# awslabs/palace

Measured on AMD Instinct MI355X. Metric: curl-curl Mult DOF/s + PCG iters/s, p=3 H(curl) 10M DOF @1/2/4/8 GPU, higher is better.
Workload: dtype f64

## Files before the change

palace_amd/csrc/pa_capi.hip:

```cpp
#include <algorithm>
#include <atomic>
#include <cmath>
#include <cstdlib>
#include <cstring>

#include "pa_hex_core.hpp"

namespace pa {

static thread_local std::string g_error;
void set_error(const std::string &msg) { g_error = msg; }

static void require_device() {
  int n = 0;
  const hipError_t err = hipGetDeviceCount(&n);
  if (err != hipSuccess || n == 0)
    throw Error(std::string("no HIP device visible: libpalace_amd has no CPU fallback (hipGetDeviceCount: ") +
                hipGetErrorString(err) + ", " + std::to_string(n) + " devices)");
}

void parse_coeff(const void *blob, size_t bytes, int dim, CoeffHost &out, size_t slot_offset) {
  const size_t nslots = bytes / 8;
  const unsigned char *base = static_cast<const unsigned char *>(blob);
  auto slot_int = [&](size_t i) {
// ... 1171 lines not shown

int pa_op_mult_essential(pa_op *op, const double *x, double *y, void *stream) {
  return guarded([&] {
    PA_REQUIRE(op && op->has_essential, "pa_op_set_essential has not been called");
    apply(op, x, y, true, (hipStream_t)stream, true);
  });
}

int pa_op_mult_essential_diag(pa_op *op, const double *x, double *y, int diag_policy, void *stream, int *handled) {
  return guarded([&] {
    PA_REQUIRE(op && op->has_essential && handled, "pa_op_set_essential has not been called");
    if (op->subs.empty() && op->msubs.empty() && op->dsubs.size() == 1 && op->dsubs[0]->d_ess_flag && x != y &&
        !TransposeScope::active()) {
      const DenseSub &ds = *op->dsubs[0];
      launch_dense_apply(ds, x, true, (hipStream_t)stream);
      launch_dense_gather(ds, y, false, (hipStream_t)stream, nullptr, nullptr, x, diag_policy ? 1 : 0);
      *handled = 1;
      return;
    }
    const SubOp *s0 = op->subs.size() == 1 ? op->subs[0] : nullptr;
    const bool fuse = s0 && op->dsubs.empty() && op->msubs.empty() &&
                      (s0->fe_type == PA_FE_HCURL  ? nd_hex_fuses_essential(*s0)
                       : s0->fe_type == PA_FE_HDIV ? s0->d_shared_bc != nullptr
                                                   : (s0->d_idxc && s0->stream_default && s0->d_perm_s_bc));
    apply(op, x, y, true, (hipStream_t)stream, true, fuse ? (diag_policy ? 1 : 0) : -1);
    *handled = fuse ? 1 : 0;
  });
}

int pa_op_prepare_fused_step(pa_op *op, int *available) {
  return guarded([&] {
    PA_REQUIRE(op && available, "null argument");
    *available = 0;
    const bool enabled = !(getenv("PALACE_AMD_FUSED_STEP") && atoi(getenv("PALACE_AMD_FUSED_STEP")) == 0);
    if (!enabled || !op->has_essential || !op->msubs.empty()) return;
    if (op->subs.empty() && op->dsubs.size() == 1) {
      *available = dense_fused_step_ok(*op->dsubs[0]) ? 1 : 0;
      return;
    }
    if (op->subs.empty() && op->dsubs.size() > 1) {
      const char *e = getenv("PALACE_AMD_FUSED_STEP_SURFACE");
      if ((e && e[0] == '0') || !dense_fused_step_ok(*op->dsubs[0]) || op->dsubs[0]->d_rows) return;
      for (size_t k = 1; k < op->dsubs.size(); k++)
        if (!op->dsubs[k]->d_rows || !op->dsubs[k]->d_idx_bc) return;
      if (!op->d_t_extra) {
        std::vector<int32_t> rows;
        for (size_t k = 1; k < op->dsubs.size(); k++) {
          std::vector<int32_t> r((size_t)op->dsubs[k]->n_rows);
          if (!r.empty()) PA_HIP(hipMemcpy(r.data(), op->dsubs[k]->d_rows, r.size() * sizeof(int32_t), hipMemcpyDeviceToHost));
          rows.insert(rows.end(), r.begin(), r.end());
        }
        std::sort(rows.begin(), rows.end());
        rows.erase(std::unique(rows.begin(), rows.end()), rows.end());
        op->n_extra_rows = (int)rows.size();
        op->d_extra_rows = dev_upload(rows.data(), std::max<size_t>(rows.size(), 1));
        if (op->dsubs.size() - 1 <= (size_t)kMaxSurfaceBlocks) {
          std::vector<int32_t> uptr(rows.size() + 1, 0), uent;
          std::vector<uint8_t> ublk;
          std::vector<std::vector<int32_t>> tptr(op->dsubs.size()), tent(op->dsubs.size());
          for (size_t k = 1; k < op->dsubs.size(); k++) {
            const DenseSub &d = *op->dsubs[k];
            tptr[k].resize((size_t)d.lsize + 1), tent[k].resize((size_t)d.ne * d.P);
            PA_HIP(hipMemcpy(tptr[k].data(), d.d_tptr, tptr[k].size() * sizeof(int32_t), hipMemcpyDeviceToHost));
            PA_HIP(hipMemcpy(tent[k].data(), d.d_tent, tent[k].size() * sizeof(int32_t), hipMemcpyDeviceToHost));
          }
          for (size_t i = 0; i < rows.size(); i++) {
            for (size_t k = 1; k < op->dsubs.size(); k++)
              for (int32_t a = tptr[k][(size_t)rows[i]]; a < tptr[k][(size_t)rows[i] + 1]; a++) uent.push_back(tent[k][(size_t)a]), ublk.push_back((uint8_t)(k - 1));
            uptr[i + 1] = (int32_t)uent.size();
          }
          op->d_urow_ptr = dev_upload(uptr.data(), uptr.size());
          op->d_uent = dev_upload(uent.data(), std::max<size_t>(uent.size(), 1));
          op->d_ublk = dev_upload(ublk.data(), std::max<size_t>(ublk.size(), 1));
        }
        op->d_t_extra = dev_alloc<double>((size_t)op->height);
        PA_HIP(hipMemset(op->d_t_extra, 0, sizeof(double) * (size_t)op->height));
      }
      *available = 1;
      return;
    }
    if (op->subs.size() != 1 || !op->dsubs.empty()) return;
    SubOp *so = op->subs[0];
    if (so->fe_type == PA_FE_H1) {
      if (!so->d_idxc || !so->stream_default || !so->d_perm_s_bc || !h1_hex_stream_ok(*so)) return;
    } else if (so->fe_type != PA_FE_HCURL || (so->q1d != 4 && so->q1d != 5) || !so->d_idxc || !so->d_perm_s_bc || !nd_hex_stream_ok(*so)) {
      return;
    }
    *available = stream_build_all(*so) ? 1 : 0;
  });
}

static const double *dense_surface_terms(pa_op *op, const double *x, hipStream_t s) {
  if (op->dsubs.size() < 2) return nullptr;
  PA_REQUIRE(op->d_t_extra, "pa_op_prepare_fused_step has not been called (or found no fused form)");
  if (op->d_urow_ptr) {
    SurfaceYe ye{};
    for (size_t k = 1; k < op->dsubs.size(); k++) {
      launch_dense_apply(*op->dsubs[k], x, true, s);
      ye.ye[k - 1] = op->dsubs[k]->d_ye;
    }
    launch_surface_rows(op->d_extra_rows, op->n_extra_rows, op->d_urow_ptr, op->d_uent, op->d_ublk, ye, op->d_t_extra, s);
    return op->d_t_extra;
  }
  launch_zero_rows(op->d_t_extra, op->d_extra_rows, op->n_extra_rows, s);
  for (size_t k = 1; k < op->dsubs.size(); k++) {
    launch_dense_apply(*op->dsubs[k], x, true, s);
    launch_dense_gather(*op->dsubs[k], op->d_t_extra, true, s);
  }
  return op->d_t_extra;
}

int pa_op_mult_cheb_step(pa_op *op, const double *x, const pa_cheb_step *step, int diag_policy, void *stream) {
  return guarded([&] {
    PA_REQUIRE(op && x && step && step->dinv && step->r0 && step->out, "null argument");
    PA_REQUIRE(x != step->out, "the step cannot overwrite its own input");
    PA_REQUIRE(!TransposeScope::active() || op->symmetric(), "transposed step of a non-symmetric operator");
    if (op->subs.empty() && !op->dsubs.empty() && dense_fused_step_ok(*op->dsubs[0])) {
      const DenseSub &ds = *op->dsubs[0];
      const double *t_add = dense_surface_terms(op, x, (hipStream_t)stream);
      launch_dense_apply(ds, x, true, (hipStream_t)stream);
      launch_dense_gather_step(ds, x, GatherStep{step->sd, step->sr, step->dinv, step->r0, step->e_prev, step->out, step->add, nullptr, 1,
                                                nullptr, nullptr, t_add},
                               diag_policy ? 1 : 0, (hipStream_t)stream);
      return;
    }
    PA_REQUIRE(op->subs.size() == 1 && op->subs[0]->n_all > 0, "pa_op_prepare_fused_step has not been called (or found no fused form)");
    const SubOp &so = *op->subs[0];
    launch_nd_hex_stream_all(so, x, (hipStream_t)stream);
    launch_et_run_gather_step(so, x, GatherStep{step->sd, step->sr, step->dinv, step->r0, step->e_prev, step->out, step->add, nullptr, 1},
                              diag_policy ? 1 : 0, (hipStream_t)stream);
  });
}

int pa_op_mult_residual(pa_op *op, const double *y, const double *b, double *res, const double *dinv, double c0, double *d0,
                        int diag_policy, void *stream) {
  return guarded([&] {
    PA_REQUIRE(op && y && b && (res || d0) && (!d0 || dinv), "null argument");
    PA_REQUIRE(y != res && y != d0, "the residual cannot overwrite the operator's input");
    PA_REQUIRE(!TransposeScope::active() || op->symmetric(), "transposed step of a non-symmetric operator");
    if (op->subs.empty() && !op->dsubs.empty() && dense_fused_step_ok(*op->dsubs[0])) {
      const DenseSub &ds = *op->dsubs[0];
      const double *t_add = dense_surface_terms(op, y, (hipStream_t)stream);
      launch_dense_apply(ds, y, true, (hipStream_t)stream);
      launch_dense_gather_step(ds, y, GatherStep{0.0, c0, dinv, b, nullptr, d0, 0, res, 2, nullptr, nullptr, t_add}, diag_policy ? 1 : 0,
                               (hipStream_t)stream);
      return;
    }
    PA_REQUIRE(op->subs.size() == 1 && op->subs[0]->n_all > 0, "pa_op_prepare_fused_step has not been called (or found no fused form)");
    const SubOp &so = *op->subs[0];
    launch_nd_hex_stream_all(so, y, (hipStream_t)stream);
    launch_et_run_gather_step(so, y, GatherStep{0.0, c0, dinv, b, nullptr, d0, 0, res, 2}, diag_policy ? 1 : 0, (hipStream_t)stream);
  });
}

int pa_op_supports_split(const pa_op *op) {
  if (!op || !op->msubs.empty()) return 0;
  if (op->subs.size() == 1 && op->dsubs.empty()) {
    const SubOp &so = *op->subs[0];
    return (nd_hex_stream_split_ok(so) || (so.fe_type == PA_FE_H1 && so.d_idxc)) ? 1 : 0;
  }
  if (op->subs.empty() && op->dsubs.size() == 1) return dense_split_ok(*op->dsubs[0]) ? 1 : 0;
  return 0;
}

int pa_op_mult_split(pa_op *op, const double *x, const double *xg0, const double *xg1, const unsigned long long *sel, double *y,
                     double *yg, int n_true, int ess_policy, void *stream) {
  return guarded([&] {
// ... 1 lines not shown
    PA_REQUIRE(pa_op_supports_split(op), "the operator has no split-vector form (pa_op_supports_split)");
    PA_REQUIRE(x != y, "in-place apply is not supported");
    PA_REQUIRE(!TransposeScope::active() || op->symmetric(), "transposed split apply of a non-symmetric operator");
    const bool masked = ess_policy >= 0;
    const SplitIO io{n_true, xg0, xg1, sel, yg};
    hipStream_t s = (hipStream_t)stream;
    if (!op->dsubs.empty()) {
      DenseSub *ds = op->dsubs[0];
      PA_REQUIRE(!masked || op->has_essential, "pa_op_set_essential has not been called");
      launch_dense_apply(*ds, x, masked, s, &io);
      launch_dense_gather(*ds, y, false, s, nullptr, &io, x, ess_policy);
      return;
    }
    SubOp *so = op->subs[0];
    PA_REQUIRE(!masked || (op->has_essential && so->d_perm_s_bc), "pa_op_set_essential has not been called");
    if (so->fe_type == PA_FE_H1)
      launch_h1_hex_stream(*so, x, y, masked, s, &io);
    else
      launch_nd_hex_stream(*so, x, y, masked, s, &io);
    launch_et_run_gather(*so, y, false, s, x, masked, ess_policy, nullptr, &io);
  });
}

int pa_op_mult_split_step(pa_op *op, const double *x, const double *xg0, const double *xg1, const unsigned long long *sel, double *yg,
                          int n_true, int ess_policy, const pa_split_step *st, void *stream) {
  return guarded([&] {
    PA_REQUIRE(op && x && xg0 && yg && st && st->r0 && st->iface_mask && st->t_iface, "null argument");
    PA_REQUIRE(st->mode == 1 ? (st->dinv && st->out) : (st->mode == 2 && (st->res || st->out) && (!st->out || st->dinv)), "invalid step");
    PA_REQUIRE(x != st->out && x != st->res, "the step cannot overwrite the operator's input");
    PA_REQUIRE(!TransposeScope::active() || op->symmetric(), "transposed split apply of a non-symmetric operator");
    PA_REQUIRE(ess_policy < 0 || op->has_essential, "pa_op_set_essential has not been called");
    const SplitIO io{n_true, xg0, xg1, sel, yg};
    hipStream_t s = (hipStream_t)stream;
    if (op->subs.empty() && op->dsubs.size() == 1 && dense_fused_step_ok(*op->dsubs[0]) && dense_split_ok(*op->dsubs[0])) {
      const DenseSub &ds = *op->dsubs[0];
      launch_dense_apply(ds, x, ess_policy >= 0, s, &io);
      launch_dense_gather_step(ds, x, GatherStep{st->sd, st->sr, st->dinv, st->r0, st->e_prev, st->out, st->add, st->res, st->mode,
                                                 st->iface_mask, st->t_iface}, ess_policy, s, &io);
      return;
    }
    PA_REQUIRE(op->subs.size() == 1 && op->dsubs.empty() && op->subs[0]->n_all > 0,
               "pa_op_prepare_fused_step has not been called (or found no fused form)");
    const SubOp &so = *op->subs[0];
    launch_nd_hex_stream_all(so, x, s, &io);
    launch_et_run_gather_step(so, x, GatherStep{st->sd, st->sr, st->dinv, st->r0, st->e_prev, st->out, st->add, st->res, st->mode,
                                                st->iface_mask, st->t_iface}, ess_policy, s, &io);
  });
}

int pa_op_mult2(pa_op *op, const double *x0, const double *x1, double *y0, double *y1, void *stream) {
  return guarded([&] { apply2(op, x0, x1, y0, y1, (hipStream_t)stream, false, -1); });
}

int pa_op_mult2_essential_diag(pa_op *op, const double *x0, const double *x1, double *y0, double *y1, int diag_policy,
                               void *stream, int *handled) {
  return guarded([&] {
    PA_REQUIRE(op && op->has_essential && handled, "pa_op_set_essential has not been called");
    *handled = apply2(op, x0, x1, y0, y1, (hipStream_t)stream, true, diag_policy ? 1 : 0) ? 1 : 0;
  });
}

int pa_op_assemble_diagonal(pa_op *op, double *diag, void *stream) {
  return guarded([&] {
    PA_REQUIRE(op && diag, "null argument");
    PA_REQUIRE(op->msubs.empty(), "mixed-space operators have no diagonal");
    PA_HIP(hipMemsetAsync(diag, 0, sizeof(double) * (size_t)op->height, (hipStream_t)stream));
    for (const SubOp *so : op->subs) {
      if (so->fe_type == PA_FE_HCURL)
        launch_nd_hex_diag(*so, diag, (hipStream_t)stream);
      else if (so->fe_type == PA_FE_HDIV)
        launch_rt_hex_diag(*so, diag, (hipStream_t)stream);
      else
        launch_h1_hex_diag(*so, diag, (hipStream_t)stream);
    }
    for (const DenseSub *ds : op->dsubs) launch_dense_diag(*ds, diag, (hipStream_t)stream);
  });
}

int pa_op_stream_affine(const pa_op *op, int32_t out[3]) {
  return guarded([&] {
    PA_REQUIRE(op && out, "null argument");
    out[0] = out[1] = out[2] = 0;
    for (const SubOp *so : op->subs)
      if (so->fe_type == PA_FE_HCURL && so->qd) {
        out[0] = so->ne, out[1] = so->qd->n_aff_elems, out[2] = so->qd->d_aff ? so->qd->n_aff_batch_elems : 0;
        return;
      }
  });
}
int pa_op_dense_gather_form(const pa_op *op, int32_t out[2]) {
  return guarded([&] {
    PA_REQUIRE(op && out, "null argument");
    out[0] = out[1] = 0;
    if (!op->dsubs.empty()) out[0] = op->dsubs[0]->ye_rows ? 1 : 0, out[1] = dense_gather_group(*op->dsubs[0]);
  });
}
int pa_op_num_sub(const pa_op *op) { return op ? (int)(op->subs.size() + op->dsubs.size() + op->msubs.size()) : -1; }
int pa_op_destroy_assembly_data(const pa_op *op) {
  return guarded([&] { PA_REQUIRE(op, "null operator"); });
}
int pa_op_height(const pa_op *op) { return op ? op->height : -1; }
int pa_op_width(const pa_op *op) { return op ? op->width : -1; }

double pa_op_algorithmic_bytes(const pa_op *op) {
  if (!op) return 0.0;
  double bytes = 0.0;
  for (const SubOp *so : op->subs) {
    if (so->fe_type == PA_FE_HDIV) {
      const bool use_v = so->qf != PA_QF_L2_1;
      const int rows = so->qd ? so->qd->ncomp : (use_v ? 11 : 2);
      bytes += (double)so->ne * ((double)so->Q * rows * 8 + (double)so->P * 6);
      continue;
    }
    bytes += (double)so->ne * ((double)so->Q * 11 * 8 + (double)so->P * (so->fe_type == PA_FE_H1 ? 4 : 5));
  }
  for (const DenseSub *ds : op->dsubs)
    bytes += (double)ds->ne * ((double)ds->Q * ds->geom->nrows * 8 + (double)ds->P * (ds->d_co ? 7 : 5));
  for (const MixedSub *ms : op->msubs)
    if (ms->hex1) bytes += (double)ms->ne * ((double)ms->Q * 11 * 8 + (double)(ms->hex1->P + ms->hex2->P) * 6);
  return bytes + 8.0 * op->height + 8.0 * op->width;
}

void pa_op_destroy(pa_op *op) {
  if (!op) return;
  for (SubOp *so : op->subs) free_sub(so);
  for (DenseSub *ds : op->dsubs) free_dense_sub(ds);
  for (MixedSub *ms : op->msubs) free_mixed_sub(ms);
  (void)hipFree(op->d_t_extra), (void)hipFree(op->d_extra_rows);
  (void)hipFree(op->d_urow_ptr), (void)hipFree(op->d_uent), (void)hipFree(op->d_ublk);
  delete op;
}

}
```

palace_amd/csrc/pa_h1_hex_stream.hip:

```cpp
#include <string>

#include "pa_hex_core.hpp"

namespace pa {

namespace {

using streamhost::kIdxWords;
constexpr int kIdxStart0 = streamhost::kIdxStart0H1;

constexpr int kH1StreamWaves = 2;

template <int P1>
struct H1StreamTab {
  double Bc[2 * (P1 + 1)];
  double Gc[2 * (P1 + 1)];
};

template <int P1>
struct H1StreamArgs {
  int ne, nbatch, chunk;
  const uint32_t *idxc;
  const uint32_t *perm;
  const double *qdata;
  const double *x;
  double *y, *ye;
  int nsplit;
  const double *xg0, *xg1;
  const unsigned long long *xg_sel;
  double *yg;
  H1StreamTab<P1> tab;
};

template <int P1, bool USE_V, bool USE_G, int MINW, bool SPLIT = false>
__global__ __launch_bounds__(64 * kH1StreamWaves, MINW) void h1_hex_stream_kernel(const H1StreamArgs<P1> a) {
  using L = H1Layout<P1, 4>;
  constexpr int Q1 = 4, NC = P1 + 1, PP = NC * NC * NC, NPL = (PP + 15) / 16, NPK = (NPL + 3) / 4;
  constexpr int NG = (USE_V ? 1 : 0) + (USE_G ? 6 : 0);
  constexpr int LDS_SIDE = (PP + 1) / 2 + (NPK + 1) * 8;
  constexpr int LDS_ELEM = (L::ELEM_PAD + LDS_SIDE + 14 + 15) / 32 * 32 + 16;
  extern __shared__ __attribute__((aligned(16))) double smem[];
  const int lane = threadIdx.x & 63;
  const int wave = __builtin_amdgcn_readfirstlane(threadIdx.x >> 6);
  const int xcd = blockIdx.x & 7;
  const int base = xcd * a.chunk, bend = min(base + a.chunk, a.nbatch);
  const int stride = (int)(gridDim.x >> 3) * kH1StreamWaves;
  int b = base + (int)(blockIdx.x >> 3) * kH1StreamWaves + wave;
  if (b >= bend) return;
  const double *Bc = a.tab.Bc, *Gc = a.tab.Gc;
  const double *xgh = nullptr;
  if (SPLIT) xgh = ((a.xg_sel ? *a.xg_sel : 0ull) & 1ull) ? a.xg1 : a.xg0;

  auto load_idx = [&](const int bb, const int sub, const int t, int (&s)[NPL + 2], unsigned (&p)[NPK + 1]) {
    const int e = bb * 4 + sub;
    const uint32_t *ic = a.idxc + (size_t)e * kIdxWords;
#pragma unroll
    for (int r = 0; r < NPL; r++) s[r] = (int)__builtin_nontemporal_load(&ic[r]);
    s[NPL] = (int)__builtin_nontemporal_load(&ic[kIdxStart0 + t]);
    s[NPL + 1] = (int)__builtin_nontemporal_load(&ic[kIdxStart0 + 16 + min(t, 11)]);
    const uint32_t *pp = a.perm + (size_t)e * ((NPK + 1) * 16) + t;
#pragma unroll
    for (int k = 0; k <= NPK; k++) p[k] = __builtin_nontemporal_load(&pp[16 * k]);
  };
  auto gather = [&](int (&s)[NPL + 2], const unsigned (&p)[NPK + 1], double (&xv)[NPL], int *stab, const int t) {
    stab[t] = s[NPL];
    if (t < 12) stab[16 + t] = s[NPL + 1];
    wave_sync();
    const unsigned fw = p[NPK];
#pragma unroll
    for (int r = 0; r < NPL; r++) {
      const unsigned w = (unsigned)s[r], low = (w & 0xffffu) & ((2u << t) - 1u);
      const int rid = (int)((w >> 16) & 31u) + __popc(low) - 1;
      const int pos = low ? 16 * r + 31 - __clz((int)low) : (int)((w >> 21) & 255u);
      int dof = stab[rid] + (t + 16 * r - pos);
      if (!(16 * r + 15 < PP) && t + 16 * r >= PP) dof = 0;
      xv[r] = SPLIT ? (dof < a.nsplit ? a.x : xgh)[dof] : a.x[dof];
      s[r] = dof | ((fw >> (2 * r + 1)) & 1u ? kExclBit : 0) | ((fw >> (18 + r)) & 1u ? kEssBit : 0);
    }
  };
  auto settle = [&](unsigned (&p)[NPK + 1]) {
#pragma unroll
    for (int k = 0; k <= NPK; k++) asm volatile("" : "+v"(p[k]));
  };
  int sA[NPL + 2];
  unsigned pA[NPK + 1];
  double xv[NPL];
  load_idx(b, lane >> 4, lane & 15, sA, pA);
  gather(sA, pA, xv, reinterpret_cast<int *>(smem + (size_t)(wave * 4 + (lane >> 4)) * LDS_ELEM + L::ELEM_PAD + LDS_SIDE), lane & 15);
#pragma unroll
  for (int r = 0; r < NPL; r++) asm volatile("" : "+v"(xv[r]));
  settle(pA);

  for (;;) {
    int lo = lane;
    asm volatile("" : "+v"(lo));
    const int sub = lo >> 4, t = lo & 15, ta = t & 3, tb = t >> 2;
    double *sm = smem + (size_t)(wave * 4 + sub) * LDS_ELEM;
    int *side = reinterpret_cast<int *>(sm + L::ELEM_PAD);
    int *stab = side + 2 * LDS_SIDE;
    const int e = b * 4 + sub;

    double gd[Q1][NG > 0 ? NG : 1];
    {
      const double *g = a.qdata + (size_t)e * NG * 64 + t;
#pragma unroll
      for (int qz = 0; qz < Q1; qz++)
#pragma unroll
        for (int c = 0; c < NG; c++) gd[qz][c] = __builtin_nontemporal_load(&g[c * 64 + 16 * qz]);
    }
    const int bn = b + stride;
    const bool more = bn < bend;
    int sB[NPL + 2];
    unsigned pB[NPK + 1];
    load_idx(more ? bn : b, sub, t, sB, pB);
    __builtin_amdgcn_sched_barrier(0);

#pragma unroll
    for (int r = 0; r < NPL; r++) {
      if (16 * r + 15 < PP || t + 16 * r < PP) {
        const int sv = sA[r];
        sm[(pA[r >> 2] >> (8 * (r & 3))) & 255u] = (sv & kEssBit) ? 0.0 : xv[r];
        side[t + 16 * r] = sv;
      }
    }
#pragma unroll
    for (int k = 0; k <= NPK; k++) side[2 * ((PP + 1) / 2) + 16 * k + t] = (int)pA[k];
    wave_sync();
    double u[NC];
    {
      const bool act = ta < NC && tb < NC;
#pragma unroll
      for (int i = 0; i < NC; i++) u[i] = act ? sm[i + NC * (ta + NC * tb)] : 0.0;
    }
    wave_sync();

    double V[Q1], GV[3][Q1];
    {
      const bool act = ta < NC && tb < NC;
#pragma unroll
      for (int qx = 0; qx < Q1; qx++) {
        double v = 0.0, d = 0.0;
#pragma unroll
        for (int i = 0; i < NC; i++) {
          v += half_even<NC, Q1>(Bc, qx, i) * u[i];
          if (USE_G) d += half_odd<NC, Q1>(Gc, qx, i) * u[i];
        }
        if (act) {
          sm[L::ia(0, qx, ta, tb)] = v;
          if (USE_G) sm[L::ia(1, qx, ta, tb)] = d;
        }
      }
    }
    wave_sync();
    {
      const bool act = tb < NC;
      double v[NC], d[NC];
#pragma unroll
      for (int j = 0; j < NC; j++) {
        v[j] = sm[L::ia(0, ta, j, act ? tb : 0)];
        if (USE_G) d[j] = sm[L::ia(1, ta, j, act ? tb : 0)];
      }
#pragma unroll
      for (int qy = 0; qy < Q1; qy++) {
        double vv = 0.0, vd = 0.0, dv = 0.0;
#pragma unroll
        for (int j = 0; j < NC; j++) {
          vv += half_even<NC, Q1>(Bc, qy, j) * v[j];
          if (USE_G) vd += half_odd<NC, Q1>(Gc, qy, j) * v[j];
          if (USE_G) dv += half_even<NC, Q1>(Bc, qy, j) * d[j];
        }
        if (act) {
          sm[L::ib(0, ta, qy, tb)] = vv;
          if (USE_G) sm[L::ib(1, ta, qy, tb)] = vd, sm[L::ib(2, ta, qy, tb)] = dv;
        }
      }
    }
    wave_sync();
    {
      double vv[NC], vd[NC], dv[NC];
#pragma unroll
      for (int k = 0; k < NC; k++) {
        vv[k] = sm[L::ib(0, ta, tb, k)];
        if (USE_G) vd[k] = sm[L::ib(1, ta, tb, k)], dv[k] = sm[L::ib(2, ta, tb, k)];
      }
#pragma unroll
      for (int qz = 0; qz < Q1; qz++) {
        double val = 0.0, dz = 0.0, dy = 0.0, dx = 0.0;
#pragma unroll
        for (int k = 0; k < NC; k++) {
          if (USE_V) val += half_even<NC, Q1>(Bc, qz, k) * vv[k];
          if (USE_G) {
            dz += half_odd<NC, Q1>(Gc, qz, k) * vv[k];
            dy += half_even<NC, Q1>(Bc, qz, k) * vd[k];
            dx += half_even<NC, Q1>(Bc, qz, k) * dv[k];
          }
        }
        V[qz] = val, GV[0][qz] = dx, GV[1][qz] = dy, GV[2][qz] = dz;
      }
    }
    wave_sync();

#pragma unroll
    for (int qz = 0; qz < Q1; qz++) {
      if (USE_V) V[qz] *= gd[qz][0];
      if (USE_G) sym_mv(&gd[qz][USE_V ? 1 : 0], GV[0][qz], GV[1][qz], GV[2][qz], GV[0][qz], GV[1][qz], GV[2][qz]);
    }

    {
#pragma unroll
      for (int k = 0; k < NC; k++) {
        double vv = 0.0, vd = 0.0, dv = 0.0;
#pragma unroll
        for (int qz = 0; qz < Q1; qz++) {
          if (USE_V) vv += half_even<NC, Q1>(Bc, qz, k) * V[qz];
          if (USE_G) {
            vv += half_odd<NC, Q1>(Gc, qz, k) * GV[2][qz];
            vd += half_even<NC, Q1>(Bc, qz, k) * GV[1][qz];
            dv += half_even<NC, Q1>(Bc, qz, k) * GV[0][qz];
          }
        }
        sm[L::ib(0, ta, tb, k)] = vv;
        if (USE_G) sm[L::ib(1, ta, tb, k)] = vd, sm[L::ib(2, ta, tb, k)] = dv;
      }
    }
    wave_sync();
    double xB[NPL];
    __builtin_amdgcn_sched_barrier(0);
    gather(sB, pB, xB, stab, t);
    settle(pB);
    __builtin_amdgcn_sched_barrier(0);
    {
      const bool act = tb < NC;
      double vv[Q1], vd[Q1], dv[Q1];
#pragma unroll
      for (int qy = 0; qy < Q1; qy++) {
        vv[qy] = sm[L::ib(0, ta, qy, act ? tb : 0)];
        if (USE_G) vd[qy] = sm[L::ib(1, ta, qy, act ? tb : 0)], dv[qy] = sm[L::ib(2, ta, qy, act ? tb : 0)];
      }
#pragma unroll
      for (int j = 0; j < NC; j++) {
        double v = 0.0, d = 0.0;
#pragma unroll
        for (int qy = 0; qy < Q1; qy++) {
          v += half_even<NC, Q1>(Bc, qy, j) * vv[qy];
          if (USE_G) v += half_odd<NC, Q1>(Gc, qy, j) * vd[qy];
          if (USE_G) d += half_even<NC, Q1>(Bc, qy, j) * dv[qy];
        }
        if (act) {
          sm[L::ia(0, ta, j, tb)] = v;
          if (USE_G) sm[L::ia(1, ta, j, tb)] = d;
        }
      }
    }
    wave_sync();
    {
      const bool act = ta < NC && tb < NC;
      double v[Q1], d[Q1];
#pragma unroll
      for (int qx = 0; qx < Q1; qx++) {
        v[qx] = sm[L::ia(0, qx, act ? ta : 0, act ? tb : 0)];
        if (USE_G) d[qx] = sm[L::ia(1, qx, act ? ta : 0, act ? tb : 0)];
      }
#pragma unroll
      for (int i = 0; i < NC; i++) {
        double r = 0.0;
#pragma unroll
        for (int qx = 0; qx < Q1; qx++) {
          r += half_even<NC, Q1>(Bc, qx, i) * v[qx];
          if (USE_G) r += half_odd<NC, Q1>(Gc, qx, i) * d[qx];
        }
        u[i] = r;
      }
    }
    wave_sync();
    {
      const bool act = ta < NC && tb < NC;
#pragma unroll
      for (int i = 0; i < NC; i++)
        if (act) sm[i + NC * (ta + NC * tb)] = u[i];
    }
    wave_sync();
#pragma unroll
    for (int r = 0; r < NPL; r++) {
      const int m = (16 * r + 15 < PP) ? t + 16 * r : min(t + 16 * r, PP - 1), mt = m & 15, mr = m >> 4;
      const unsigned fl = (unsigned)side[2 * ((PP + 1) / 2) + 16 * NPK + mt] >> (2 * mr);
      const double v = sm[((unsigned)side[2 * ((PP + 1) / 2) + 16 * (mr >> 2) + mt] >> (8 * (mr & 3))) & 255u];
      const int d = side[m] & (kExclBit - 1);
      double *yd = a.y;
      if (SPLIT) yd = d < a.nsplit ? a.y : a.yg;
      double *dst = (fl & 2u) ? yd + d : a.ye + ((size_t)e * PP + m);
      *dst = v;
    }
    wave_sync();
    if (!more) break;
    b = bn;
#pragma unroll
    for (int r = 0; r < NPL; r++) sA[r] = sB[r], xv[r] = xB[r];
#pragma unroll
    for (int k = 0; k <= NPK; k++) pA[k] = pB[k];
  }
}

int device_cus_h1() {
  static int cus = [] {
    int dev = 0, n = 0;
    if (hipGetDevice(&dev) != hipSuccess || hipDeviceGetAttribute(&n, hipDeviceAttributeMultiprocessorCount, dev) != hipSuccess || n <= 0)
      n = 256;
    return n;
  }();
  return cus;
}

template <int P1, bool V, bool G, bool SPLIT = false>
void launch_vg(const SubOp &so, H1StreamArgs<P1> &a, hipStream_t s) {
  using L = H1Layout<P1, 4>;
  constexpr int MINW = 3;
  constexpr int NC = P1 + 1, PP = NC * NC * NC, NPL = (PP + 15) / 16, NPK = (NPL + 3) / 4;
  for (int i = 0; i < 2 * NC; i++) a.tab.Bc[i] = so.Bc[i], a.tab.Gc[i] = so.Gc[i];
  const size_t lds = sizeof(double) * (size_t)(kH1StreamWaves * 4) * ((L::ELEM_PAD + (PP + 1) / 2 + (NPK + 1) * 8 + 14 + 15) / 32 * 32 + 16);
  static const int per_cu = [&] {
    int nb = 0;
    if (hipOccupancyMaxActiveBlocksPerMultiprocessor(&nb, h1_hex_stream_kernel<P1, V, G, MINW, SPLIT>, 64 * kH1StreamWaves, lds) != hipSuccess ||
        nb <= 0)
      nb = 2;
    return std::max(1, std::min(std::min(nb, MINW * 2), 8));
  }();
  a.nbatch = (so.ne + 3) / 4;
  a.chunk = (a.nbatch + 7) / 8;
  const int cus = device_cus_h1();
  int grid = std::max(8, std::min(per_cu * cus, ((a.nbatch + kH1StreamWaves - 1) / kH1StreamWaves + 7) / 8 * 8));
  grid = (grid + 7) / 8 * 8;
  hipLaunchKernelGGL((h1_hex_stream_kernel<P1, V, G, MINW, SPLIT>), dim3(grid), dim3(64 * kH1StreamWaves), lds, s, a);
  PA_HIP(hipGetLastError());
}

template <int P1>
void launch_p(const SubOp &so, const double *x, double *y, bool masked, hipStream_t s, const SplitIO *split, bool all) {
  H1StreamArgs<P1> a;
  a.ne = so.ne;
  a.idxc = so.d_idxc;
  a.perm = all ? so.d_perm_s_all : (masked ? so.d_perm_s_bc : so.d_perm_s);
  a.qdata = so.qd->d;
  a.x = x, a.y = y, a.ye = so.d_ye;
  a.nsplit = -1, a.xg0 = a.xg1 = nullptr, a.xg_sel = nullptr, a.yg = nullptr;
  if (split) {
    PA_REQUIRE(split->n_true >= 0 && split->n_true <= so.lsize, "split point outside the local vector");
    a.nsplit = split->n_true;
    a.xg0 = split->xg0 - split->n_true, a.xg1 = (split->xg1 ? split->xg1 : split->xg0) - split->n_true;
    a.xg_sel = split->sel, a.yg = split->yg - split->n_true;
    switch (so.qf) {
      case PA_QF_HCURL_33: launch_vg<P1, false, true, true>(so, a, s); break;
      case PA_QF_H1_1: launch_vg<P1, true, false, true>(so, a, s); break;
      case PA_QF_HCURLMASS_33: launch_vg<P1, true, true, true>(so, a, s); break;
      default: throw Error("QFunction not available for H1 hexahedra");
    }
    return;
  }
  switch (so.qf) {
    case PA_QF_HCURL_33: launch_vg<P1, false, true>(so, a, s); break;
    case PA_QF_H1_1: launch_vg<P1, true, false>(so, a, s); break;
    case PA_QF_HCURLMASS_33: launch_vg<P1, true, true>(so, a, s); break;
    default: throw Error("QFunction not available for H1 hexahedra");
  }
}

}

bool h1_hex_stream_capable(const SubOp &so) {
  static const bool enabled = [] {
    const char *e = getenv("PALACE_AMD_STREAM"), *h = getenv("PALACE_AMD_STREAM_H1");
    return !(e && e[0] == '0') && !(h && h[0] == '0');
  }();
  return enabled && so.fe_type == PA_FE_H1 && so.q1d == 4 && so.p >= 1 && so.p <= 3 && so.qd && so.qd->d && so.d_ye && so.d_tptr;
}

bool h1_hex_stream_ok(const SubOp &so) {
  static const bool enabled = [] {
    const char *e = getenv("PALACE_AMD_STREAM"), *h = getenv("PALACE_AMD_STREAM_H1");
    return !(e && e[0] == '0') && !(h && h[0] == '0');
  }();
  if (!enabled) return false;
  static const bool all = [] {
    const char *h = getenv("PALACE_AMD_STREAM_H1");
    return h && std::string(h) == "all";
  }();
  return so.fe_type == PA_FE_H1 && so.q1d == 4 && so.p >= (all ? 1 : 3) && so.p <= 3 && so.qd && so.qd->d && so.d_ye && so.d_tptr;
}

void launch_h1_hex_stream(const SubOp &so, const double *x, double *y, bool masked, hipStream_t s, const SplitIO *split, bool all) {
  switch (so.p) {
    case 1: launch_p<1>(so, x, y, masked, s, split, all); break;
    case 2: launch_p<2>(so, x, y, masked, s, split, all); break;
    case 3: launch_p<3>(so, x, y, masked, s, split, all); break;
    default: throw Error("no streaming H1 kernel for this order");
  }
}

}
```

palace_amd/csrc/pa_nd_hex_stream.hip:

```cpp
#include <algorithm>
#include <map>

#include "pa_nd_hex_core.hpp"

#ifndef PA_CPLX_QAHEAD
#define PA_CPLX_QAHEAD 0
#endif
#ifndef PA_STREAM_QAHEAD
#define PA_STREAM_QAHEAD 0
#endif
#ifndef PA_KM_MINW_LOW
#define PA_KM_MINW_LOW 2
#endif
#ifndef PA_KM_MINW
#define PA_KM_MINW 2
#endif

namespace pa {

typedef double d2v __attribute__((ext_vector_type(2)));

#ifdef PA_STREAM_TRACE
constexpr int kTraceWG = 64, kTraceBatches = 14, kTraceStamps = 12;
__device__ unsigned long long g_trace[kTraceWG * kTraceBatches * kTraceStamps];
// ... 534 lines not shown
#pragma unroll
    for (int u = 0; u < kGatherILP; u++)
#pragma unroll
      for (int q = 0; q < 4; q++) w[u][q] = pos[u][q] >= 0 ? p2.ye1[(size_t)pos[u][q] + j[u]] : 0.0;
#pragma unroll
    for (int u = 0; u < kGatherILP; u++) {
      s1[u] = (live[u] && fix[u] && ess_policy) ? p2.x1[d[u]] : 0.0;
#pragma unroll
      for (int q = 0; q < 4; q++) s1[u] += w[u][q];
      if (live[u])
        for (int p = h[u].ptr + 4; p < pe[u]; p++) s1[u] += p2.ye1[(size_t)rpos[p] + j[u]];
      if (live[u]) p2.y1[d[u]] = s1[u];
    }
  }
#pragma unroll
  for (int u = 0; u < kGatherILP; u++) {
#pragma unroll
    for (int q = 0; q < 4; q++) s[u] += v[u][q];
    if (live[u])
      for (int p = h[u].ptr + 4; p < pe[u]; p++) s[u] += ye[(size_t)rpos[p] + j[u]];
  }
  if (STEP) {
#pragma unroll
    for (int u = 0; u < kGatherILP; u++) {
      if (!live[u]) continue;
      if (d[u] >= nsplit) {
        yg[d[u]] = s[u];
        continue;
      }
      if (st.iface_mask && (st.iface_mask[d[u]] & 2)) {
        st.t_iface[d[u]] = s[u];
        continue;
      }
      const double rv = sr0[u] - s[u];
      if (st.mode == 2) {
        if (st.res) st.res[d[u]] = rv;
        if (st.out) st.out[d[u]] = st.sr * sdi[u] * rv;
        continue;
      }
      double dk = st.sr * sdi[u] * rv;
      dk += st.sd * (se[u] - sep[u]);
      st.out[d[u]] = so[u] + (se[u] + dk);
    }
    return;
  }
#pragma unroll
  for (int u = 0; u < kGatherILP; u++)
    if (live[u]) (d[u] < nsplit ? y : yg)[d[u]] = yold[u] + s[u];
}

bool nd_hex_stream_ok(const SubOp &so) {
  static const bool enabled = !(getenv("PALACE_AMD_STREAM") && atoi(getenv("PALACE_AMD_STREAM")) == 0);
  if (!enabled) return false;
  if (so.q1d == 5) return nd_hex_stream5_ok(so);
  if (so.fe_type != PA_FE_HCURL || so.q1d != 4 || so.p > 3 || !so.qd || !so.d_ye || !so.d_perm_x) return false;
  return so.qd->metric || so.qd->ncomp == 6 || (so.qd->ncomp == 12 && so.qf == PA_QF_HDIVMASS_33);
}

static bool wide_form(const SubOp &so) { return so.fe_type == PA_FE_HCURL && so.q1d == 5; }

void stream_element_coefficients(SubOp &so) {
  if (so.d_coef_s) return;
  const int ne = so.ne, nep = (ne + 3) & ~3;
  const std::vector<int32_t> &attr = so.geom->h_attr;
  PA_REQUIRE((int)attr.size() == ne, "element attributes missing");
  const CoeffHost *cm = nullptr, *cc = nullptr;
  if (so.qf == PA_QF_HDIV_33) cc = &so.c0;
  if (so.qf == PA_QF_HCURL_33) cm = &so.c0;
  if (so.qf == PA_QF_HDIVMASS_33) cm = &so.c0, cc = &so.c1;
  auto value = [&](const CoeffHost *c, int at) {
    if (!c) return 0.0;
    int k = 0;
    if (!c->attr_mat.empty()) {
      PA_REQUIRE(at >= 1 && at <= (int)c->attr_mat.size(), "element attribute outside the coefficient's attribute map");
      k = c->attr_mat[at - 1];
    }
    return c->mat[(size_t)9 * k];
  };
  std::vector<double> coef((size_t)nep * 2, 0.0);
  for (int e = 0; e < ne; e++) coef[2 * (size_t)e] = value(cm, attr[e]), coef[2 * (size_t)e + 1] = value(cc, attr[e]);
  so.d_coef_s = dev_upload(coef.data(), coef.size());
}

__global__ __launch_bounds__(64) void stream_affine_kernel(const int ne, const int ncomp, const int metric, const double *__restrict__ qd,
                                                           const double w0, const double w1, const double tol,
                                                           double *__restrict__ aff, unsigned char *__restrict__ flag) {
  const int e = blockIdx.x, q = threadIdx.x;
  if (e >= ne) return;
  auto w1d = [&](const int i) { return (i == 0 || i == 3) ? w0 : w1; };
  const double wq = w1d(q & 3) * w1d((q >> 2) & 3) * w1d(q >> 4);
  auto wave_sum = [](double v) {
    for (int m = 32; m >= 1; m >>= 1) v += __shfl_xor(v, m, 64);
    return v;
  };
  auto wave_max = [](double v) {
    for (int m = 32; m >= 1; m >>= 1) v = fmax(v, __shfl_xor(v, m, 64));
    return v;
  };
  bool ok = true;
  for (int g0 = 0; g0 < ncomp; g0 += 6) {
    const int gn = min(6, ncomp - g0);
    double mean[6], dev = 0.0, scale = 0.0;
    for (int c = 0; c < gn; c++) {
      const double v = qd[(size_t)e * ncomp * 64 + nd_qd_offset(4, g0 + c, q)];
      const double r = (metric && g0 + c == 6) ? v * wq : v / wq;
      mean[c] = wave_sum(r) * (1.0 / 64.0);
      dev = fmax(dev, wave_max(fabs(r - mean[c])));
      scale = fmax(scale, fabs(mean[c]));
    }
    ok = ok && dev <= tol * scale;
    if (q < 2 * gn) {
      const int c = q >> 1, h = q & 1;
      const bool inv = metric && g0 + c == 6;
      double *row = aff + ((size_t)e * 2 * ncomp + 2 * (g0 + c) + h) * 2;
      double m = 0.0;
      for (int k = 0; k < 6; k++) m = (k == c) ? mean[k] : m;
      row[0] = inv ? m / w1d(2 * h) : m * w1d(2 * h);
      row[1] = inv ? m / w1d(2 * h + 1) : m * w1d(2 * h + 1);
    }
  }
  if (q == 0) flag[e] = ok ? 1 : 0;
}

static void stream_affine_setup(SubOp &so) {
  QData &qd = *so.qd;
  if (qd.aff_done) return;
  qd.aff_done = true;
  const bool enabled = !(getenv("PALACE_AMD_STREAM_AFFINE") && atoi(getenv("PALACE_AMD_STREAM_AFFINE")) == 0);
  if (!enabled || so.q1d != 4 || (int)so.geom->w1.size() != 4) return;
  const std::vector<double> &w = so.geom->w1;
  if (w[0] != w[3] || w[1] != w[2]) return;
  const int ne = so.ne, nep = (ne + 3) & ~3;
  const size_t nrow = (size_t)nep * 2 * qd.ncomp * 2;
  double *d_aff = nullptr;
  unsigned char *d_flag = nullptr;
  PA_HIP(hipMalloc(&d_aff, nrow * sizeof(double)));
  PA_HIP(hipMemset(d_aff, 0, nrow * sizeof(double)));
  PA_HIP(hipMalloc(&d_flag, (size_t)nep));
  PA_HIP(hipMemset(d_flag, 0, (size_t)nep));
  const double tol = getenv("PALACE_AMD_AFFINE_TOL") ? atof(getenv("PALACE_AMD_AFFINE_TOL")) : 1e-13;
  hipLaunchKernelGGL(stream_affine_kernel, dim3(ne), dim3(64), 0, nullptr, ne, qd.ncomp, qd.metric ? 1 : 0, qd.d, w[0], w[1], tol, d_aff,
                     d_flag);
  PA_HIP(hipGetLastError());
  std::vector<unsigned char> flag((size_t)nep, 0);
  PA_HIP(hipMemcpy(flag.data(), d_flag, (size_t)nep, hipMemcpyDeviceToHost));
  (void)hipFree(d_flag);
  qd.batch_aff.assign((size_t)nep / 4, 0);
  for (int e = 0; e < ne; e++) qd.n_aff_elems += flag[e];
  for (int b = 0; b < nep / 4; b++)
    if (flag[4 * b] && flag[4 * b + 1] && flag[4 * b + 2] && flag[4 * b + 3]) qd.batch_aff[b] = 1, qd.n_aff_batch_elems += 4;
  if (qd.n_aff_batch_elems == 0) {
    (void)hipFree(d_aff);
    qd.batch_aff.clear();
    return;
  }
  qd.d_aff = d_aff;
  qd.wq2[0] = w[0], qd.wq2[1] = w[1];
}

void build_stream(SubOp &so) {
  if (so.d_idxc || !(nd_hex_stream_ok(so) || h1_hex_stream_capable(so))) return;
  const int P = so.P, ne = so.ne;
  std::vector<uint32_t> ic, pp;
  if (wide_form(so)) {
    if (!streamhost::pack_index_wide(ne, P, so.lsize, so.h_sidx.data(), so.h_perm.data(), ic, pp)) return;
  } else if (!streamhost::pack_index(ne, P, so.lsize, so.h_sidx.data(), so.h_perm.data(), ic, pp,
                                     so.fe_type == PA_FE_H1 ? streamhost::kIdxStart0H1 : streamhost::kIdxStart0))
    return;
#ifdef PA_ABLATION
  const int price_group = (so.fe_type == PA_FE_HCURL && !wide_form(so) && getenv("PALACE_AMD_PRICE_BLOCK")) ? atoi(getenv("PALACE_AMD_PRICE_BLOCK")) : 0;
#else
  constexpr int price_group = 0;
#endif
  if (price_group > 1) {
    const size_t nnz = (size_t)ne * P;
    const int npl = (P + 15) / 16, npk = (npl + 3) / 4;
    so.h_price_skip.assign(nnz, 0);
    std::vector<int32_t> seen((size_t)so.lsize, -1), cnt((size_t)so.lsize, 0), cnt2((size_t)so.lsize, 0);
    for (size_t k = 0; k < nnz; k++) {
      const int d = streamhost::dof_of(so.h_sidx[k]), g = (int)(k / P) / price_group;
      cnt[d]++;
      if (seen[d] == g) so.h_price_skip[k] = 1; else seen[d] = g, cnt2[d]++;
    }
    size_t dropped = 0, freed = 0;
    for (size_t k = 0; k < nnz; k++) {
      const int d = streamhost::dof_of(so.h_sidx[k]);
      const bool direct = so.h_price_skip[k] || (cnt2[d] == 1 && cnt[d] > 1);
      if (!direct) continue;
      const size_t e = k / P;
      const int m = (int)(k - e * P), t = m & 15, r = m >> 4;
      pp[(e * (npk + 1) + npk) * 16 + t] |= 2u << (2 * r);
      dropped += so.h_price_skip[k] ? 1 : 0, freed += so.h_price_skip[k] ? 0 : 1;
    }
    std::vector<int32_t> shared2;
    for (int d = 0; d < so.lsize; d++)
      if (cnt2[d] > 1) shared2.push_back(d);
    fprintf(stderr, "PALACE_AMD_PRICE_BLOCK=%d: %zu of %zu E-vector entries dropped, %zu more leave the gather; shared dofs %zu -> %zu\n",
            price_group, dropped, nnz, freed, so.h_shared.size(), shared2.size());
    so.h_shared = shared2;
    so.n_shared = (int)shared2.size();
  }
  if (so.fe_type == PA_FE_HCURL && !wide_form(so)) {
    stream_affine_setup(so);
    const int npl = (P + 15) / 16, npk = (npl + 3) / 4;
    for (size_t b = 0; b < so.qd->batch_aff.size(); b++)
      if (so.qd->batch_aff[b])
        for (size_t e = 4 * b; e < 4 * b + 4; e++)
          for (int t = 0; t < 16; t++) pp[(e * (npk + 1) + npk) * 16 + t] |= streamhost::kAffBit;
  }
  so.h_perm_s = pp;
  if (so.fe_type == PA_FE_HCURL && !wide_form(so)) {
    const int npl = (P + 15) / 16, npk = (npl + 3) / 4, nep = (ne + 3) & ~3, sw = npk * 16;
    std::vector<uint32_t> flagw((size_t)nep * 16), slots;
    std::map<std::vector<uint32_t>, uint32_t> dict;
    std::vector<uint32_t> key((size_t)sw);
    for (int e = 0; e < nep; e++) {
      const uint32_t *row = &pp[(size_t)e * (npk + 1) * 16];
      std::copy(row + sw, row + sw + 16, flagw.begin() + (size_t)e * 16);
      key.assign(row, row + sw);
      auto it = dict.find(key);
      if (it == dict.end()) {
        it = dict.emplace(key, (uint32_t)dict.size()).first;
        slots.insert(slots.end(), key.begin(), key.end());
      }
      ic[(size_t)e * streamhost::kIdxWords + streamhost::kIdxPattern] = it->second;
    }
    so.n_slot_patterns = (int)dict.size();
    so.d_flagw = dev_upload(flagw.data(), flagw.size());
    so.d_slots = dev_upload(slots.data(), slots.size());
  }
  so.d_idxc = dev_upload(ic.data(), ic.size());
  so.d_perm_s = dev_upload(pp.data(), pp.size());
  if (so.qd->metric || (so.iso && so.qf == PA_QF_HDIV_33 && so.geom->d_xnodes)) stream_element_coefficients(so);

  std::vector<uint32_t> code;
  std::vector<RunHdr> hdr;
  std::vector<int32_t> rpos;
  streamhost::build_runs(ne, P, so.lsize, so.h_sidx.data(), so.h_shared, code, hdr, rpos, nullptr,
                         so.h_price_skip.empty() ? nullptr : so.h_price_skip.data());
  {
    const std::vector<RunChunk> ch = streamhost::run_chunks(code);
    so.d_rchunk = dev_upload(reinterpret_cast<const uint32_t *>(ch.data()), 4 * ch.size());
  }
  so.d_rhdr = dev_upload(reinterpret_cast<const int32_t *>(hdr.data()), 2 * hdr.size());
  so.d_rpos = dev_upload(rpos.data(), rpos.size());
  so.n_runs = (int)hdr.size() - 1;
}

void stream_set_essential(SubOp &so, const std::vector<char> &flag) {
  if (!so.d_idxc) return;
  so.h_ess_flag = flag;
  if (so.n_all > 0) {
    hipFree(so.d_flagw_all), hipFree(so.d_perm_s_all), hipFree(so.d_rchunk_all), hipFree(so.d_rhdr_all), hipFree(so.d_rpos_all);
    so.d_flagw_all = so.d_perm_s_all = nullptr, so.d_rchunk_all = nullptr, so.d_rhdr_all = so.d_rpos_all = nullptr, so.n_all = 0;
  }
  const int P = so.P, npl = (P + 15) / 16, npk = (npl + 3) / 4;
  std::vector<uint32_t> pb(so.h_perm_s);
  const size_t nnz = (size_t)so.ne * so.P;
  const bool wide = wide_form(so);
  const int npkw = ((P + 31) / 32 + 1) / 2;
  for (size_t k = 0; k < nnz; k++) {
    if (flag[streamhost::dof_of(so.h_sidx[k])]) {
      const size_t e = k / P;
      if (wide) {
        const int m = (int)(k - e * P), t = m & 31, r = m >> 5;
        uint32_t &w = pb[(e * npkw + (r >> 1)) * 32 + t];
        w &= ~(streamhost::kWideExcl << (16 * (r & 1)));
        w |= streamhost::kWideEss << (16 * (r & 1));
        continue;
      }
      const int m = (int)(k - e * P), t = m & 15, r = m >> 4;
      uint32_t &fw = pb[(e * (npk + 1) + npk) * 16 + t];
      fw &= ~(2u << (2 * r));
      fw |= 1u << (18 + r);
    }
  }
  hipFree(so.d_perm_s_bc);
  so.d_perm_s_bc = dev_upload(pb.data(), pb.size());
  if (so.d_flagw) {
    const int nep = (so.ne + 3) & ~3;
    std::vector<uint32_t> fb((size_t)nep * 16);
    for (int e = 0; e < nep; e++) std::copy(&pb[((size_t)e * (npk + 1) + npk) * 16], &pb[((size_t)e * (npk + 1) + npk) * 16] + 16, fb.begin() + (size_t)e * 16);
    hipFree(so.d_flagw_bc);
    so.d_flagw_bc = dev_upload(fb.data(), fb.size());
  }
// ... 338 lines not shown
```

Before: 66.43 billion.

## Extend affine-element compressed quadrature data path to H1 hex stream kernel

Brings the affine-element detection used by the H(curl) stream kernel to the H1 stream kernel. Batches whose geometric factors are constant per element now read a small per-element table scaled by tensor-product weights instead of the full per-quadrature-point qdata, which cuts global memory traffic. The fused-step availability check for H1 also switches from stream_default/h1_hex_stream_ok to h1_hex_stream_capable, so the H1 stream path may be enabled in more cases. The cost is extra setup and a per-batch branch in the kernel. Correctness depends on the tolerance check and on weight symmetry.

```diff
diff --git a/palace_amd/csrc/pa_capi.hip b/palace_amd/csrc/pa_capi.hip
--- a/palace_amd/csrc/pa_capi.hip
+++ b/palace_amd/csrc/pa_capi.hip
@@ -1277,7 +1277,7 @@
     if (op->subs.size() != 1 || !op->dsubs.empty()) return;
     SubOp *so = op->subs[0];
     if (so->fe_type == PA_FE_H1) {
-      if (!so->d_idxc || !so->stream_default || !so->d_perm_s_bc || !h1_hex_stream_ok(*so)) return;
+      if (!so->d_idxc || !so->d_perm_s_bc || !h1_hex_stream_capable(*so)) return;
     } else if (so->fe_type != PA_FE_HCURL || (so->q1d != 4 && so->q1d != 5) || !so->d_idxc || !so->d_perm_s_bc || !nd_hex_stream_ok(*so)) {
       return;
     }
@@ -1445,7 +1445,7 @@
     PA_REQUIRE(op && out, "null argument");
     out[0] = out[1] = out[2] = 0;
     for (const SubOp *so : op->subs)
-      if (so->fe_type == PA_FE_HCURL && so->qd) {
+      if ((so->fe_type == PA_FE_HCURL || (so->fe_type == PA_FE_H1 && so->d_idxc)) && so->qd) {
         out[0] = so->ne, out[1] = so->qd->n_aff_elems, out[2] = so->qd->d_aff ? so->qd->n_aff_batch_elems : 0;
         return;
       }
diff --git a/palace_amd/csrc/pa_h1_hex_stream.hip b/palace_amd/csrc/pa_h1_hex_stream.hip
--- a/palace_amd/csrc/pa_h1_hex_stream.hip
+++ b/palace_amd/csrc/pa_h1_hex_stream.hip
@@ -23,6 +23,8 @@
   const uint32_t *idxc;
   const uint32_t *perm;
   const double *qdata;
+  const double *qaff;
+  double wq2[2];
   const double *x;
   double *y, *ye;
   int nsplit;
@@ -100,13 +102,15 @@
     int *stab = side + 2 * LDS_SIDE;
     const int e = b * 4 + sub;
 
+    const int aff = __builtin_amdgcn_readfirstlane((int)(pA[NPK] >> 31));
     double gd[Q1][NG > 0 ? NG : 1];
     {
-      const double *g = a.qdata + (size_t)e * NG * 64 + t;
+      const int cs = aff ? 4 : 64, ps = aff ? 1 : 16;
+      const double *g = aff ? a.qaff + (size_t)e * (NG * 4) : a.qdata + ((size_t)e * (NG * 64) + t);
 #pragma unroll
       for (int qz = 0; qz < Q1; qz++)
 #pragma unroll
-        for (int c = 0; c < NG; c++) gd[qz][c] = __builtin_nontemporal_load(&g[c * 64 + 16 * qz]);
+        for (int c = 0; c < NG; c++) gd[qz][c] = __builtin_nontemporal_load(&g[c * cs + ps * qz]);
     }
     const int bn = b + stride;
     const bool more = bn < bend;
@@ -200,10 +204,14 @@
     }
     wave_sync();
 
+    const double wab = aff ? ((ta == 0 || ta == 3) ? a.wq2[0] : a.wq2[1]) * ((tb == 0 || tb == 3) ? a.wq2[0] : a.wq2[1]) : 1.0;
 #pragma unroll
     for (int qz = 0; qz < Q1; qz++) {
-      if (USE_V) V[qz] *= gd[qz][0];
-      if (USE_G) sym_mv(&gd[qz][USE_V ? 1 : 0], GV[0][qz], GV[1][qz], GV[2][qz], GV[0][qz], GV[1][qz], GV[2][qz]);
+      if (USE_V) V[qz] *= gd[qz][0] * wab;
+      if (USE_G) {
+        sym_mv(&gd[qz][USE_V ? 1 : 0], GV[0][qz], GV[1][qz], GV[2][qz], GV[0][qz], GV[1][qz], GV[2][qz]);
+        GV[0][qz] *= wab, GV[1][qz] *= wab, GV[2][qz] *= wab;
+      }
     }
 
     {
@@ -341,6 +349,7 @@
   a.idxc = so.d_idxc;
   a.perm = all ? so.d_perm_s_all : (masked ? so.d_perm_s_bc : so.d_perm_s);
   a.qdata = so.qd->d;
+  a.qaff = so.qd->d_aff, a.wq2[0] = so.qd->wq2[0], a.wq2[1] = so.qd->wq2[1];
   a.x = x, a.y = y, a.ye = so.d_ye;
   a.nsplit = -1, a.xg0 = a.xg1 = nullptr, a.xg_sel = nullptr, a.yg = nullptr;
   if (split) {
diff --git a/palace_amd/csrc/pa_nd_hex_stream.hip b/palace_amd/csrc/pa_nd_hex_stream.hip
--- a/palace_amd/csrc/pa_nd_hex_stream.hip
+++ b/palace_amd/csrc/pa_nd_hex_stream.hip
@@ -640,7 +640,8 @@
   so.d_coef_s = dev_upload(coef.data(), coef.size());
 }
 
-__global__ __launch_bounds__(64) void stream_affine_kernel(const int ne, const int ncomp, const int metric, const double *__restrict__ qd,
+__global__ __launch_bounds__(64) void stream_affine_kernel(const int ne, const int ncomp, const int metric, const int h1,
+                                                           const double *__restrict__ qd,
                                                            const double w0, const double w1, const double tol,
                                                            double *__restrict__ aff, unsigned char *__restrict__ flag) {
   const int e = blockIdx.x, q = threadIdx.x;
@@ -656,18 +657,25 @@
     return v;
   };
   bool ok = true;
-  for (int g0 = 0; g0 < ncomp; g0 += 6) {
-    const int gn = min(6, ncomp - g0);
+  for (int g0 = 0, gn = 0; g0 < ncomp; g0 += gn) {
+    gn = (h1 && g0 == 0 && ncomp % 6 == 1) ? 1 : min(6, ncomp - g0);
     double mean[6], dev = 0.0, scale = 0.0;
     for (int c = 0; c < gn; c++) {
-      const double v = qd[(size_t)e * ncomp * 64 + nd_qd_offset(4, g0 + c, q)];
+      const double v = qd[(size_t)e * ncomp * 64 + (h1 ? (g0 + c) * 64 + q : nd_qd_offset(4, g0 + c, q))];
       const double r = (metric && g0 + c == 6) ? v * wq : v / wq;
       mean[c] = wave_sum(r) * (1.0 / 64.0);
       dev = fmax(dev, wave_max(fabs(r - mean[c])));
       scale = fmax(scale, fabs(mean[c]));
     }
     ok = ok && dev <= tol * scale;
-    if (q < 2 * gn) {
+    if (h1) {
+      if (q < 4 * gn) {
+        const int c = q >> 2;
+        double m = 0.0;
+        for (int k = 0; k < 6; k++) m = (k == c) ? mean[k] : m;
+        aff[((size_t)e * ncomp + g0 + c) * 4 + (q & 3)] = m * w1d(q & 3);
+      }
+    } else if (q < 2 * gn) {
       const int c = q >> 1, h = q & 1;
       const bool inv = metric && g0 + c == 6;
       double *row = aff + ((size_t)e * 2 * ncomp + 2 * (g0 + c) + h) * 2;
@@ -697,8 +705,8 @@
   PA_HIP(hipMalloc(&d_flag, (size_t)nep));
   PA_HIP(hipMemset(d_flag, 0, (size_t)nep));
   const double tol = getenv("PALACE_AMD_AFFINE_TOL") ? atof(getenv("PALACE_AMD_AFFINE_TOL")) : 1e-13;
-  hipLaunchKernelGGL(stream_affine_kernel, dim3(ne), dim3(64), 0, nullptr, ne, qd.ncomp, qd.metric ? 1 : 0, qd.d, w[0], w[1], tol, d_aff,
-                     d_flag);
+  hipLaunchKernelGGL(stream_affine_kernel, dim3(ne), dim3(64), 0, nullptr, ne, qd.ncomp, qd.metric ? 1 : 0,
+                     so.fe_type == PA_FE_H1 ? 1 : 0, qd.d, w[0], w[1], tol, d_aff, d_flag);
   PA_HIP(hipGetLastError());
   std::vector<unsigned char> flag((size_t)nep, 0);
   PA_HIP(hipMemcpy(flag.data(), d_flag, (size_t)nep, hipMemcpyDeviceToHost));
@@ -758,7 +766,7 @@
     so.h_shared = shared2;
     so.n_shared = (int)shared2.size();
   }
-  if (so.fe_type == PA_FE_HCURL && !wide_form(so)) {
+  if ((so.fe_type == PA_FE_HCURL && !wide_form(so)) || so.fe_type == PA_FE_H1) {
     stream_affine_setup(so);
     const int npl = (P + 15) / 16, npk = (npl + 3) / 4;
     for (size_t b = 0; b < so.qd->batch_aff.size(); b++)
```

Result: slower. 65.34 billion (-1.6%).
